# populationgenomics/cuKING

Hardware: AMD Instinct MI355X
Metric: sample-pairs/s (all-pairs KING) (higher is better)
Workload: dtype fp4 products, f32 accumulate (exact integers)

## Files before the change

### cuking_amd/csrc/king_common.h

```cpp
#ifndef CUKING_AMD_KING_COMMON_H_
#define CUKING_AMD_KING_COMMON_H_

#include <hip/hip_runtime.h>
#include <stdint.h>

#include "cuking_amd.h"
#include "king_submatrix.h"

namespace cuking {

constexpr uint32_t kLayoutWord = 0;
constexpr uint32_t kLayoutQuad = 1;
constexpr uint32_t kLayoutNibble = 2;
constexpr uint32_t kLayoutNibbleStats = 3;

struct PlaneGeometry {
  uint32_t num_rows, num_cols;
  uint32_t rows_padded, cols_padded;
  uint32_t col_base;
  uint32_t s_stride;
  uint32_t k_words;
  uint32_t diag;
};

// ... 65 lines not shown
  const uint32_t *tile_list_count;
  uint32_t tile_list_cap;
  const float2 *sample_stats;
  const uint4 *t2;
  uint32_t *filter_ctrl;
  unsigned long long *filter_totals;
  uint2 *cand_list;
  uint32_t cand_cap;
  uint32_t quadrant_cap;
  uint2 *dense_list;
  uint32_t dense_cap;
  uint32_t fsplit_parts, fsplit_first, fsplit_tile0;
  float4 *fsplit_slabs;
  uint32_t *fsplit_tickets;
  const uint32_t *check_steps;
  const float *prefix_u;
  const unsigned long long *cohort_sums;
  uint32_t check0, check1;
  uint32_t rotate, rotate_min_steps;
  uint32_t rotate_min_tiles;
  uint8_t *tile_done;
  const uint32_t *gate;
  uint32_t gate_count;
  const uint8_t *skip_tiles;
  uint64_t skip_base;
  const uint32_t *perm;
  uint32_t *codes_ready;
};

constexpr uint32_t kCheckEmitCap = 64;
constexpr uint32_t kNumCheckShares = 8;
constexpr uint32_t kCheckShares64[kNumCheckShares] = {8, 50, 53, 56, 58, 60, 61, 62};
constexpr uint32_t kNumPhases = 128;
constexpr uint32_t kPhasesPerShare = kNumPhases / 64;
constexpr uint32_t kNumCum = kNumPhases - 1;
__host__ __device__ inline uint32_t phase_step(uint32_t all_steps, uint32_t x) {
  return (uint32_t)((uint64_t)all_steps * x / kNumPhases);
}
__host__ __device__ inline uint32_t check_step_of(uint32_t all_steps, uint32_t k,
                                                  uint32_t min_steps = 64) {
  if (all_steps < min_steps) return 0;
  return phase_step(all_steps, kCheckShares64[k] * kPhasesPerShare);
}
constexpr uint32_t kFilterSplitSlabs = 256;
constexpr size_t kFilterSlabBytes = 256 * 256 * sizeof(float);
constexpr size_t kFilterTicketBytes = kFilterSplitSlabs * sizeof(uint32_t);
__host__ __device__ inline size_t plane_bytes(const PlaneGeometry &g,
                                              uint32_t layout) {
  const size_t base = (size_t)g.k_words * g.s_stride * (layout == kLayoutQuad ? 8 : 16);
  if (layout == kLayoutNibble) return base + base / 4;
  if (layout == kLayoutNibbleStats)
    return base + base / 4 + base / 2 + (size_t)g.s_stride * sizeof(float2) +
           (size_t)g.s_stride * kNumCum * sizeof(float) + 64 + 64 +
           64 + (size_t)g.s_stride * (4 + 8 + 4 * kNumCum + 16);
  return base;
}
__host__ __device__ inline const uint4 *plane_t2(const uint4 *planes, const PlaneGeometry &g) {
  return planes + (size_t)g.k_words * g.s_stride * 5 / 4;
}
__host__ __device__ inline const float2 *plane_stats(const uint4 *planes, const PlaneGeometry &g) {
  return reinterpret_cast<const float2 *>(planes + (size_t)g.k_words * g.s_stride * 7 / 4);
}
__host__ __device__ inline const float *plane_prefix_u(const uint4 *planes, const PlaneGeometry &g) {
  return reinterpret_cast<const float *>(plane_stats(planes, g) + g.s_stride);
}
__host__ __device__ inline const unsigned long long *plane_cohort_sums(const uint4 *planes,
                                                                       const PlaneGeometry &g) {
  return reinterpret_cast<const unsigned long long *>(plane_prefix_u(planes, g) +
                                                      (size_t)g.s_stride * kNumCum);
}

struct TiledVariant {
  const char *name;
  uint32_t tile;
  uint32_t k_chunk;
  uint32_t threads;
  uint32_t lds_bytes;
  uint32_t layout;
};

constexpr uint32_t kMfmaMaxSites = 1u << 24;

constexpr int kNumTiledVariants = 8;
constexpr int kMfmaVariant = 5;
constexpr int kMfmaN4Variant = 6;
constexpr uint32_t kMfmaN4MaxSites = 1u << 22;
constexpr int kMfmaN4Stages = 5;
constexpr uint32_t kMfmaN4LdsBytes = kMfmaN4Stages * 2 * 2 * 4 * 128 * 16;
static_assert(kMfmaN4LdsBytes <= 160 * 1024, "LDS of one CU");
constexpr int kMfmaFilterVariant = 7;
constexpr uint32_t kFilterTile = 256;
constexpr uint32_t kFilterLdsBytes = 5 * 2 * 2 * 2 * 256 * 16;
static_assert(kFilterLdsBytes <= 160 * 1024, "LDS of one CU");
constexpr uint32_t kFilterChunkTiles = 1u << 17;
constexpr uint32_t kFilterCandCap = 1u << 25;
constexpr uint32_t kFilterQuadrantCap = 384;
constexpr size_t kFilterCtrlBytes = 256;
constexpr uint32_t kCtrlCand = 0, kCtrlDense = 1, kCtrlDyn = 2, kCtrlFinished = 3,
                   kCtrlLeft = 4, kCtrlAllLeave = 5, kCtrlGate = 6;
constexpr uint32_t kCtrlStepTicks = 8, kCtrlPos = 16, kPosSlots = 16;
constexpr size_t kCtrlChunkBytes = (kCtrlPos + 8 * kPosSlots * 2) * 4;
constexpr uint32_t kTotalCand = 0, kTotalDense = 1, kTotalEarly = 2, kTotalRotated = 3;
constexpr uint32_t kNumTotals = 4;
__host__ __device__ inline const uint32_t *plane_check_steps(const uint4 *planes,
                                                             const PlaneGeometry &g) {
  return reinterpret_cast<const uint32_t *>(plane_cohort_sums(planes, g) + 8);
}
__host__ __device__ inline uint32_t *plane_flags(const uint4 *planes, const PlaneGeometry &g) {
  return const_cast<uint32_t *>(plane_check_steps(planes, g)) + 16;
}
__host__ __device__ inline uint32_t *plane_perm(const uint4 *planes, const PlaneGeometry &g) {
  return plane_flags(planes, g) + 16;
}
__host__ __device__ inline float2 *plane_tmp_stats(const uint4 *planes, const PlaneGeometry &g) {
  return reinterpret_cast<float2 *>(plane_perm(planes, g) + g.s_stride);
}
__host__ __device__ inline float *plane_tmp_prefix(const uint4 *planes, const PlaneGeometry &g) {
  return reinterpret_cast<float *>(plane_tmp_stats(planes, g) + g.s_stride);
}
__host__ __device__ inline uint32_t *plane_sort_words(const uint4 *planes, const PlaneGeometry &g) {
  return reinterpret_cast<uint32_t *>(plane_tmp_prefix(planes, g) +
                                      (size_t)g.s_stride * kNumCum);
}
constexpr uint32_t kNoSample = 0xFFFFFFFFu;

struct FilterScratchLayout {
  size_t tile_done, totals, tickets, cand, dense, slabs, bytes;
  uint32_t chunk_tiles, cand_entries;
};
inline FilterScratchLayout filter_scratch_layout(uint64_t tiles) {
  FilterScratchLayout l;
  l.chunk_tiles = (uint32_t)(tiles < kFilterChunkTiles ? (tiles ? tiles : 1) : kFilterChunkTiles);
  const uint64_t cand = (uint64_t)l.chunk_tiles * 4 * 64;
  l.cand_entries = (uint32_t)(cand < kFilterCandCap ? cand : kFilterCandCap);
  auto up = [](size_t x) { return (x + 255) / 256 * 256; };
  l.tile_done = kCtrlChunkBytes;
  l.totals = up(l.tile_done + l.chunk_tiles);
  l.tickets = l.totals + kFilterCtrlBytes;
  l.cand = l.tickets + kFilterTicketBytes;
  l.dense = l.cand + up((size_t)l.cand_entries * sizeof(uint2));
  l.slabs = l.dense + up((size_t)l.chunk_tiles * 4 * sizeof(uint2));
  l.bytes = l.slabs + kFilterSplitSlabs * kFilterSlabBytes;
  return l;
}
inline bool is_mfma_variant(int v) {
  return v == kMfmaVariant || v == kMfmaN4Variant || v == kMfmaFilterVariant;
}
constexpr int kMfmaStages = 6;
constexpr uint32_t kMfmaLdsBytes = kMfmaStages * 2 * 2 * 2 * 128 * 16;
constexpr uint32_t kMfmaParkBytes = 4 * 64 * 64 * 4;
static_assert(kMfmaLdsBytes + kMfmaParkBytes <= 160 * 1024, "LDS of one CU");
const TiledVariant &tiled_variant(int v);
hipError_t launch_tiled(int variant, bool full, const TiledArgs &args,
                        uint64_t num_tiles, hipStream_t stream);
hipError_t launch_mfma(bool full, bool nibble, const TiledArgs &args, uint64_t num_tiles,
                       uint32_t lds_bytes, hipStream_t stream);
hipError_t launch_mfma_list(const TiledArgs &args, uint32_t grid, hipStream_t stream);
hipError_t launch_mfma_gated(const TiledArgs &args, uint64_t num_units, uint32_t grid,
                             hipStream_t stream);
hipError_t launch_filter(const TiledArgs &args, uint64_t num_tiles, hipStream_t stream);
hipError_t launch_sample_stats(const uint64_t *d_bit_sets, uint32_t words_per_sample,
                               const PlaneGeometry &geo, uint4 *d_planes, uint32_t s_begin,
                               uint32_t s_end, hipStream_t stream);
void set_filter_check_min_steps(uint32_t steps);
uint32_t filter_check_min_steps();
size_t sort_temp_bytes_for(uint32_t n);
hipError_t launch_sample_order(const PlaneGeometry &geo, uint32_t words_per_sample,
                               uint4 *d_planes, uint32_t s_begin, uint32_t s_end, bool sort,
                               void *sort_temp, size_t sort_temp_bytes, hipStream_t stream);
hipError_t launch_prepare_nibbles(bool codes, bool t2, const uint64_t *d_bit_sets,
                                  uint32_t words_per_sample, const PlaneGeometry &geo,
                                  uint4 *d_planes, const uint32_t *perm, uint32_t s_tile_begin,
                                  uint32_t s_tile_end, const uint32_t *gate,
                                  const uint32_t *ready, hipStream_t stream);
hipError_t launch_mark_codes_ready(const uint32_t *gate, uint32_t *ready, hipStream_t stream);
// ... 45 lines not shown
```

### cuking_amd/csrc/king_filter.hip

```cpp
#include <hip/hip_runtime.h>
#include <stdio.h>

#include <atomic>
#include <stdlib.h>

#include "king_common.h"
#include "king_device.h"

#pragma clang diagnostic ignored "-Winline-asm"

namespace cuking {

namespace {

typedef int v8i __attribute__((ext_vector_type(8)));
typedef float v16f __attribute__((ext_vector_type(16)));

constexpr int kT = (int)kFilterTile;
constexpr int kUnits = 2;
constexpr int kStages = 5;
constexpr int kSliceU4 = kT;
constexpr int kStageU4 = 2 * 2 * kUnits * kSliceU4;
constexpr int kStageReqs = 4 * kUnits;
constexpr int kSyncVm = (kStages - 3) * kStageReqs + (kStageReqs - 2);
static_assert(kSyncVm < 64, "vmcnt is a 6-bit counter");
static_assert(kStages * kStageU4 * 16 == (int)kFilterLdsBytes, "LDS size");
constexpr int vmcnt_imm(int n) { return 0x0F70 | (n & 15) | ((n >> 4) << 14); }
constexpr uint32_t kNoPair = 0xFFFFFFFFu;

__device__ __forceinline__ uint32_t source_sample(const PlaneGeometry &geo, uint32_t ps) {
  if (geo.diag || ps < geo.rows_padded) return ps < geo.num_rows ? ps : kNoPair;
  const uint32_t c = ps - geo.col_base;
  return c < geo.num_cols ? geo.num_rows + c : kNoPair;
}

struct CheckWords {
  uint32_t w[kNumCheckShares];
};
constexpr uint32_t kStatsMaxSteps = kMfmaN4MaxSites / 256;
__global__ __launch_bounds__(256) void sample_stats_kernel(
    const uint64_t *__restrict__ bits, uint32_t words_per_sample, PlaneGeometry geo,
    float2 *__restrict__ stats, float *__restrict__ cum, unsigned long long *__restrict__ sums,
    uint32_t *__restrict__ steps_out, CheckWords cw, uint32_t s_begin, uint32_t s_end) {
  __shared__ uint8_t phase_of[kStatsMaxSteps];
  __shared__ int32_t phase_sum[4][kNumPhases];
  const uint32_t lane = threadIdx.x & 63, wave = threadIdx.x >> 6;
  if (blockIdx.x == 0 && threadIdx.x < kNumCheckShares) steps_out[threadIdx.x] = cw.w[threadIdx.x];
  const uint32_t all_steps = geo.k_words / 8;
  for (uint32_t st = threadIdx.x; st < all_steps; st += 256) {
    const uint32_t x = (kNumPhases * (st + 1) - 1) / all_steps;
    phase_of[st] = (uint8_t)(x < kNumPhases ? x : kNumPhases - 1);
  }
#pragma unroll
  for (uint32_t k = 0; k < kNumPhases / 64; ++k) phase_sum[wave][lane + 64 * k] = 0;
  __syncthreads();
  const uint32_t ps = s_begin + blockIdx.x * 4 + wave;
  if (ps >= s_end) return;
  const uint32_t src = source_sample(geo, ps);
  int32_t yc = 0, mc = 0, hc = 0;
  if (src != kNoPair) {
    const uint32_t n = words_per_sample / 2;
    const uint64_t *het = bits + (uint64_t)src * words_per_sample;
    const uint64_t *hom = het + n;
    constexpr uint32_t kAhead = 4;
    for (uint32_t w0 = 0; w0 < n; w0 += 64 * kAhead) {
      uint64_t h[kAhead], v[kAhead];
#pragma unroll
      for (uint32_t k = 0; k < kAhead; ++k) {
        const uint32_t w = w0 + 64 * k + lane;
        const bool in = w < n;
        h[k] = in ? het[w] : 0ull;
        v[k] = in ? hom[w] : 0ull;
      }
#pragma unroll
      for (uint32_t k = 0; k < kAhead; ++k) {
        const uint32_t w = w0 + 64 * k + lane;
        const bool in = w < n;
        const int32_t y = in ? __popcll(~h[k]) : 0;
        const int32_t m = __popcll(h[k] & v[k]);
        yc += y;
        mc += m;
        hc += __popcll(h[k] & ~v[k]);
        int32_t d = y - m;
        d += __shfl_xor(d, 1);
        d += __shfl_xor(d, 2);
        if ((lane & 3) == 0 && in) atomicAdd(&phase_sum[wave][phase_of[w >> 2]], d);
      }
    }
#pragma unroll
    for (int off = 32; off > 0; off >>= 1) {
      yc += __shfl_xor(yc, off);
      mc += __shfl_xor(mc, off);
      hc += __shfl_xor(hc, off);
    }
  }
  static_assert(kNumPhases == 128, "two phases per lane");
  const int32_t p0 = phase_sum[wave][2 * lane], p1 = phase_sum[wave][2 * lane + 1];
  int32_t run = p0 + p1;
#pragma unroll
  for (int off = 1; off < 64; off <<= 1) {
    const int32_t up = __shfl_up(run, off);
    if ((int)lane >= off) run += up;
  }
  cum[(size_t)(2 * lane) * geo.s_stride + ps] = (float)(run - p1);
  if (2 * lane + 1 < kNumCum) cum[(size_t)(2 * lane + 1) * geo.s_stride + ps] = (float)run;
  if (lane == 0) {
    stats[ps] = make_float2((float)(yc - mc), (float)hc);
    if (src != kNoPair && ((blockIdx.x & 15) == 0 || gridDim.x < 64)) {
      __hip_atomic_fetch_add(sums, 1ull, __ATOMIC_RELAXED, __HIP_MEMORY_SCOPE_AGENT);
      __hip_atomic_fetch_add(sums + 1, (unsigned long long)mc, __ATOMIC_RELAXED,
                             __HIP_MEMORY_SCOPE_AGENT);
      __hip_atomic_fetch_add(sums + 2, (unsigned long long)hc, __ATOMIC_RELAXED,
                             __HIP_MEMORY_SCOPE_AGENT);
    }
  }
}

__device__ __forceinline__ v16f mma(const v8i a, const v8i b, const v16f c) {
  return __builtin_amdgcn_mfma_scale_f32_32x32x64_f8f6f4(a, b, c, 4 , 4, 0, 0, 0, 0);
}

__device__ __forceinline__ v8i tfrag(const uint4 w, uint32_t mask) {
  v8i r = {0, 0, 0, 0, 0, 0, 0, 0};
  r[0] = (int)(w.x & mask);
  r[1] = (int)(w.y & mask);
  r[2] = (int)(w.z & mask);
  r[3] = (int)(w.w & mask);
  return r;
}

__device__ __forceinline__ uint4 shl2(const uint4 w) {
  return make_uint4(w.x << 2, w.y << 2, w.z << 2, w.w << 2);
}

#define F_ISSUE(SRC, DST, OFF)                                                 \
  asm volatile("s_mov_b32 m0, %0\n\t"                                          \
               "s_nop 0\n\t"                                                   \
               "global_load_lds_dwordx4 %1, %2 offset:" #OFF                   \
               :                                                               \
               : "s"(DST), "v"(lane16), "s"(SRC)                               \
               : "memory", "m0")

__device__ __forceinline__ int filter_tile(const TiledArgs &a, const uint32_t wg, uint4 *const lds) {
  uint32_t bid = wg;
  const bool split = a.fsplit_parts != 0 && wg >= a.fsplit_first;
  uint32_t part = 0, piece = 0;
  if (split) {
    piece = wg - a.fsplit_first;
    part = __builtin_amdgcn_readfirstlane(piece % a.fsplit_parts);
    bid = a.fsplit_tile0 + piece / a.fsplit_parts;
  } else
  if (a.dyn_tiles != 0 && wg >= a.launch_tiles) {
    uint32_t *slot = reinterpret_cast<uint32_t *>(lds);
    if (threadIdx.x == 0)
      *slot = __hip_atomic_fetch_add(a.filter_ctrl + kCtrlDyn, 1u, __ATOMIC_RELAXED,
                                     __HIP_MEMORY_SCOPE_AGENT);
    __syncthreads();
    const uint32_t t = __builtin_amdgcn_readfirstlane(*slot);
    __syncthreads();
    if (t >= a.dyn_tiles) return 1;
    bid = a.launch_tiles + t;
  } else if (a.xcd_chunk == 1) {
    const uint32_t x = bid & 7, j = bid >> 3;
    bid = (((j >> 5) * 8 + x) << 5) + (j & 31);
    if (bid >= a.launch_tiles) return 0;
  }
  bid = __builtin_amdgcn_readfirstlane(bid);
  uint32_t tr, tc;
  if (!decode_tile_space(a, a.tile_begin + bid, &tr, &tc)) return 0;
  tr = __builtin_amdgcn_readfirstlane(tr);
  tc = __builtin_amdgcn_readfirstlane(tc);

  const uint32_t lane = threadIdx.x & 63;
  const uint32_t wave = __builtin_amdgcn_readfirstlane(threadIdx.x >> 6);
  const uint32_t wy = wave >> 1, wx = wave & 1;
  uint32_t xcd_pos = 0;
  if (!split && a.tile_done != nullptr) {
    uint32_t *verdict = reinterpret_cast<uint32_t *>(lds);
    if (threadIdx.x == 0) {
      uint32_t leave = __hip_atomic_load(a.filter_ctrl + kCtrlAllLeave, __ATOMIC_RELAXED,
                                         __HIP_MEMORY_SCOPE_AGENT);
      if (leave == 0 && a.cohort_sums != nullptr && a.check_steps != nullptr) {
        const float ns = (float)a.cohort_sums[0], nm = (float)a.cohort_sums[1],
                    nh = (float)a.cohort_sums[2];
        if (ns > 0.f && nh > 0.f) {
// ... 16 lines not shown
        const uint32_t finished = __hip_atomic_load(a.filter_ctrl + kCtrlFinished, __ATOMIC_RELAXED,
                                                    __HIP_MEMORY_SCOPE_AGENT);
        if (finished >= 512 && 2 * dense_so_far > finished) {
          leave = 1;
          __hip_atomic_store(a.filter_ctrl + kCtrlAllLeave, 1u, __ATOMIC_RELAXED,
                             __HIP_MEMORY_SCOPE_AGENT);
          __hip_atomic_store(a.filter_ctrl + kCtrlGate, 1u, __ATOMIC_RELAXED,
                             __HIP_MEMORY_SCOPE_AGENT);
        }
      }
      verdict[0] = leave;
    }
    if (a.rotate == 1 && threadIdx.x < kPosSlots) {
      const uint32_t x = wg & 7;
      const unsigned long long said = __hip_atomic_load(
          reinterpret_cast<const unsigned long long *>(a.filter_ctrl + kCtrlPos) + x * kPosSlots +
              threadIdx.x,
          __ATOMIC_RELAXED, __HIP_MEMORY_SCOPE_AGENT);
      const uint32_t ticks16 = __hip_atomic_load(a.filter_ctrl + kCtrlStepTicks + x,
                                                 __ATOMIC_RELAXED, __HIP_MEMORY_SCOPE_AGENT);
      uint32_t pos = (uint32_t)(said >> 32);
      const uint32_t ago = (uint32_t)__builtin_amdgcn_s_memrealtime() - (uint32_t)said;
      if (said != 0 && ticks16 != 0 && ago < 16384u)
        pos += ago * 16u / ticks16;
      verdict[1 + threadIdx.x] = pos;
    }
    __syncthreads();
    const bool give_up = verdict[0] != 0;
    if (a.rotate == 1) {
#pragma unroll
      for (uint32_t k = 0; k < kPosSlots; ++k) xcd_pos = max(xcd_pos, verdict[1 + k]);
    }
    __syncthreads();
    if (give_up) {
      if (threadIdx.x == 0)
        __hip_atomic_fetch_add(a.filter_totals + kTotalDense, 4ull, __ATOMIC_RELAXED,
                               __HIP_MEMORY_SCOPE_AGENT);
      return 0;
    }
  }
  xcd_pos = __builtin_amdgcn_readfirstlane(xcd_pos);
  const uint32_t g = lane >> 5;
  const uint32_t lr = lane & 31;
  uint32_t lane16 = lane * 16;
  const uint32_t s_stride = a.geo.s_stride;
  const uint32_t all_steps = a.geo.k_words / (4 * kUnits);
  const uint32_t k_first = __builtin_amdgcn_readfirstlane(
      split ? part * all_steps / a.fsplit_parts : 0u);
  const uint32_t num_steps = __builtin_amdgcn_readfirstlane(
      split ? (part + 1) * all_steps / a.fsplit_parts - k_first : all_steps);
  const uint4 *g_rows = a.t2 + (uint64_t)tr * kT;
  const uint4 *g_cols = a.t2 + a.geo.col_base + (uint64_t)tc * kT;

  uint32_t mT;
  asm volatile("s_mov_b32 %0, 0xcccccccc" : "=s"(mT));

  const uint32_t dma_side = wave >> 1, dma_h = wave & 1;
  const uint32_t row_bytes = s_stride * 16;
  const char *const g_wave = reinterpret_cast<const char *>(
      (dma_side ? g_cols : g_rows) + ((uint64_t)2 * kUnits * k_first + kUnits * dma_h) * s_stride);
  const uint32_t l_wave = (uint32_t)(uintptr_t)(lds_void_ptr)(
      lds + ((dma_side * 2 + dma_h) * kUnits) * kSliceU4);
  struct Addr { const char *src; uint32_t dst; };
  const uint32_t kstep_bytes = 2 * kUnits * row_bytes;
  const char *seg_src = g_wave;
  uint32_t seg_steps = num_steps;
  uint32_t seg_wrap = 0xFFFFFFFFu;
  auto addr_of = [&](uint32_t step, uint32_t buf) {
    Addr pa;
    if (step >= seg_steps) step = seg_steps - 1;
    const int32_t rel = (int32_t)step - (int32_t)(step >= seg_wrap ? all_steps : 0u);
    pa.src = seg_src + (int64_t)rel * (int64_t)kstep_bytes;
    pa.dst = l_wave + buf * (kStageU4 * 16);
    asm volatile("" : "+s"(pa.src), "+s"(pa.dst));
    return pa;
  };
  auto addr_next = [&](const Addr &cur, uint32_t step, uint32_t buf) {
    Addr pa;
    const int32_t adv = (int32_t)(step < seg_steps ? 1u : 0u) -
                        (int32_t)(step == seg_wrap ? all_steps : 0u);
    pa.src = cur.src + (int64_t)adv * (int64_t)kstep_bytes;
    pa.dst = l_wave + buf * (kStageU4 * 16);
    asm volatile("" : "+s"(pa.src), "+s"(pa.dst));
    return pa;
  };
#define F_ISSUE4(PA, C)                                                        \
  {                                                                            \
    const char *src_ = (PA).src + (C) * row_bytes;                             \
    const uint32_t dst_ = (PA).dst + (C) * (kSliceU4 * 16);                    \
    F_ISSUE(src_, dst_, 0);                                                    \
    F_ISSUE(src_, dst_, 1024);                                                 \
    F_ISSUE(src_, dst_, 2048);                                                 \
    F_ISSUE(src_, dst_, 3072);                                                 \
  }

  v16f acc[4][4];
#pragma unroll
  for (int bi = 0; bi < 4; ++bi)
#pragma unroll
    for (int bj = 0; bj < 4; ++bj)
#pragma unroll
      for (int r = 0; r < 16; ++r) acc[bi][bj][r] = 0.f;

  uint32_t row_off = ((0 * 2 + g) * kUnits) * kSliceU4 + wy * 128 + lr;
  uint32_t col_off = ((1 * 2 + g) * kUnits) * kSliceU4 + wx * 128 + lr;
  asm volatile("" : "+v"(row_off), "+v"(col_off), "+v"(lane16));
  v8i FA[2][4], FB[2][4];
  uint4 RAW[8];
#define F_READ(K, BUF, C)                                                      \
  RAW[K] = lds[(BUF) * kStageU4 + ((K) < 4 ? row_off : col_off) + (C) * kSliceU4 + ((K) & 3) * 32];
#define F_PIN4(W) asm volatile("" : "+v"((W).x), "+v"((W).y), "+v"((W).z), "+v"((W).w));
#define F_PINF(F) asm volatile("" : "+v"((F)[0]), "+v"((F)[1]), "+v"((F)[2]), "+v"((F)[3]));
#define F_BUILD_B(NXT, K)                                                      \
  F_PIN4(RAW[K])                                                               \
  if ((K) < 4) {                                                               \
    FA[NXT][(K) & 3] = tfrag(RAW[K], mT);                                      \
    F_PINF(FA[NXT][(K) & 3])                                                   \
  } else {                                                                     \
    FB[NXT][(K) & 3] = tfrag(RAW[K], mT);                                      \
    F_PINF(FB[NXT][(K) & 3])                                                   \
  }
#define F_BUILD_A(NXT, K)                                                      \
  F_PIN4(RAW[K])                                                               \
  if ((K) < 4) {                                                               \
    FA[NXT][(K) & 3] = tfrag(shl2(RAW[K]), mT);                                \
    F_PINF(FA[NXT][(K) & 3])                                                   \
  } else {                                                                     \
    FB[NXT][(K) & 3] = tfrag(shl2(RAW[K]), mT);                                \
    F_PINF(FB[NXT][(K) & 3])                                                   \
  }
#define F_MMA(CUR, BI, BJ) acc[BI][BJ] = mma(FA[CUR][BI], FB[CUR][BJ], acc[BI][BJ]);
#define F_BAR __builtin_amdgcn_sched_barrier(0);
#define F_SLICE_B(CUR, NXT, PA, DC, OFF0, OFF1)                                \
  {                                                                            \
    const char *src_ = (PA).src + (DC) * row_bytes;                            \
    const uint32_t dst_ = (PA).dst + (DC) * (kSliceU4 * 16);                   \
    F_ISSUE(src_, dst_, OFF0);                                                 \
    F_MMA(CUR, 0, 0) F_BAR                                                     \
    F_BUILD_A(NXT, 0) F_MMA(CUR, 0, 1) F_BAR                                   \
    F_MMA(CUR, 0, 2) F_BAR                                                     \
    F_BUILD_A(NXT, 1) F_MMA(CUR, 0, 3) F_BAR                                   \
    F_MMA(CUR, 1, 0) F_BAR                                                     \
    F_BUILD_A(NXT, 2) F_MMA(CUR, 1, 1) F_BAR                                   \
    F_MMA(CUR, 1, 2) F_BAR                                                     \
    F_BUILD_A(NXT, 3) F_MMA(CUR, 1, 3) F_BAR                                   \
    F_ISSUE(src_, dst_, OFF1);                                                 \
    F_MMA(CUR, 2, 0) F_BAR                                                     \
    F_BUILD_A(NXT, 4) F_MMA(CUR, 2, 1) F_BAR                                   \
    F_MMA(CUR, 2, 2) F_BAR                                                     \
    F_BUILD_A(NXT, 5) F_MMA(CUR, 2, 3) F_BAR                                   \
    F_MMA(CUR, 3, 0) F_BAR                                                     \
    F_BUILD_A(NXT, 6) F_MMA(CUR, 3, 1) F_BAR                                   \
    F_MMA(CUR, 3, 2) F_BAR                                                     \
    F_BUILD_A(NXT, 7) F_MMA(CUR, 3, 3) F_BAR                                   \
  }
#define F_SLICE_A(CUR, NXT, RBUF, RC, SYNC, PA, DC, OFF0, OFF1)                \
  {                                                                            \
    if (SYNC) {                                                                \
      __builtin_amdgcn_s_waitcnt(vmcnt_imm(kSyncVm));                          \
      __syncthreads();                                                         \
    }                                                                          \
    const char *src_ = (PA).src + (DC) * row_bytes;                            \
    const uint32_t dst_ = (PA).dst + (DC) * (kSliceU4 * 16);                   \
    F_READ(0, RBUF, RC) F_READ(1, RBUF, RC)                                    \
    F_ISSUE(src_, dst_, OFF0);                                                 \
    F_MMA(CUR, 0, 0) F_MMA(CUR, 0, 1) F_BAR                                    \
    F_READ(2, RBUF, RC) F_READ(3, RBUF, RC)                                    \
    F_MMA(CUR, 0, 2) F_MMA(CUR, 0, 3) F_BAR                                    \
    F_READ(4, RBUF, RC) F_READ(5, RBUF, RC)                                    \
    F_ISSUE(src_, dst_, OFF1);                                                 \
    F_MMA(CUR, 1, 0) F_MMA(CUR, 1, 1) F_BAR                                    \
    F_READ(6, RBUF, RC) F_READ(7, RBUF, RC)                                    \
    F_MMA(CUR, 1, 2) F_MMA(CUR, 1, 3) F_BAR                                    \
    F_BUILD_B(NXT, 0) F_MMA(CUR, 2, 0) F_BAR                                   \
    F_BUILD_B(NXT, 1) F_MMA(CUR, 2, 1) F_BAR                                   \
    F_BUILD_B(NXT, 2) F_MMA(CUR, 2, 2) F_BAR                                   \
    F_BUILD_B(NXT, 3) F_MMA(CUR, 2, 3) F_BAR                                   \
    F_BUILD_B(NXT, 4) F_MMA(CUR, 3, 0) F_BAR                                   \
    F_BUILD_B(NXT, 5) F_MMA(CUR, 3, 1) F_BAR                                   \
    F_BUILD_B(NXT, 6) F_MMA(CUR, 3, 2) F_BAR                                   \
    F_BUILD_B(NXT, 7) F_MMA(CUR, 3, 3) F_BAR                                   \
  }
#define F_KSTEP                                                                \
  {                                                                            \
// ... 24 lines not shown
        phase = (bid * 37u + 11u) & (kNumPhases - 1);
      } else {
        phase = (a.rotate - 3u) & (kNumPhases - 1);
      }
      k0 = phase_step(all_steps, phase);
      start_abs = base + k0;
      wrap = k0 != 0 ? all_steps - k0 : 0u;
    }
    float kappa = -1.f;
    {
      const float ns = (float)a.cohort_sums[0], nm = (float)a.cohort_sums[1],
                  nh = (float)a.cohort_sums[2];
      if (ns > 0.f && nh > 0.f) {
        const float sites = 256.f * (float)all_steps;
        const float m = nm / (ns * sites), h = nh / (ns * sites);
        kappa = m * (1.f + m / (2.f * h * (1.f - m))) + 4.6f * rsqrtf(sites) + 0.003f;
      }
    }
    auto steps_of = [&](uint32_t share) {
      const uint32_t hi = phase + share * kPhasesPerShare;
      return hi <= kNumPhases ? phase_step(all_steps, hi) - k0
                              : (all_steps - k0) + phase_step(all_steps, hi - kNumPhases);
    };
    if ((a.check0 == 2 || (a.check0 == 1 && kappa > 0.7f * a.kin_threshold)) &&
        a.check_steps[0] != 0)
      chk0 = steps_of(kCheckShares64[0]);
    const uint32_t sw1 = a.check1 & 0xFFu;
    if (sw1 >= 2) {
      entry1 = sw1 - 2;
    } else if (sw1 == 1 && kappa >= 0.f) {
      const float f64 = 64.f * (1.f - 2.f * a.kin_threshold) / (1.f - 2.f * kappa);
      if (f64 <= 62.f) {
        share1 = (uint32_t)ceilf(f64);
        if (share1 < 32) share1 = 32;
        entry1 = 1;
      }
    }
#pragma unroll
    for (uint32_t k = 1; k < kNumCheckShares; ++k)
      if (sw1 >= 2 && k == entry1) share1 = kCheckShares64[k];
    if (share1 != 0 && a.check_steps[entry1] != 0) chk1 = steps_of(share1);
    if (chk0 >= num_steps) chk0 = 0;
    if (chk1 >= num_steps || chk1 <= chk0) chk1 = 0;
  }
  chk0 = __builtin_amdgcn_readfirstlane(chk0);
  chk1 = __builtin_amdgcn_readfirstlane(chk1);
  share1 = __builtin_amdgcn_readfirstlane(share1);
  phase = __builtin_amdgcn_readfirstlane(phase);
  k0 = __builtin_amdgcn_readfirstlane(k0);
  wrap = __builtin_amdgcn_readfirstlane(wrap);
  start_abs = __builtin_amdgcn_readfirstlane(start_abs);
  auto prefix_u_of = [&](uint32_t share, size_t idx, float total) {
    const uint32_t hi = phase + share * kPhasesPerShare;
    const uint32_t xb = hi > kNumPhases ? hi - kNumPhases : hi;
    float u = hi > kNumPhases ? total : 0.f;
    if (xb == kNumPhases)
      u += total;
    else if (xb != 0)
      u += a.prefix_u[(size_t)(xb - 1) * s_stride + idx];
    if (phase != 0) u -= a.prefix_u[(size_t)(phase - 1) * s_stride + idx];
    return u;
  };
  unsigned long long *const pos_word =
      reinterpret_cast<unsigned long long *>(a.filter_ctrl + kCtrlPos) +
      (wg & 7) * kPosSlots + ((wg >> 3) & (kPosSlots - 1));
  uint32_t *const ticks_word = a.filter_ctrl + kCtrlStepTicks + (wg & 7);
  const uint32_t t_start = a.rotate == 1 ? (uint32_t)__builtin_amdgcn_s_memrealtime() : 0u;
#define F_PUBLISH(STEPS)                                                       \
  if (a.rotate == 1 && wave == 0) {                                            \
    const uint32_t now_ = (uint32_t)__builtin_amdgcn_s_memrealtime();          \
    const unsigned long long val_ =                                            \
        ((unsigned long long)(start_abs + (STEPS)) << 32) | now_;              \
     \
    const uint32_t t16_ = (STEPS) >= 32 ? (now_ - t_start) * 16u / (STEPS) : 0u; \
    const uint32_t zero_ = 0;                                                  \
    unsigned long long save_;                                                  \
    asm volatile("s_mov_b64 %0, exec\n\t"                                      \
                 "s_mov_b64 exec, 1\n\t"                                       \
                 "global_store_dwordx2 %1, %2, %3\n\t"                         \
                 "s_mov_b64 exec, %0"                                          \
                 : "=&s"(save_)                                                \
                 : "v"(zero_), "v"(val_), "s"(pos_word)                        \
                 : "memory");                                                  \
    if (t16_ != 0)                                                             \
      asm volatile("s_mov_b64 %0, exec\n\t"                                    \
                   "s_mov_b64 exec, 1\n\t"                                     \
                   "global_store_dword %1, %2, %3\n\t"                         \
                   "s_mov_b64 exec, %0"                                        \
                   : "=&s"(save_)                                              \
                   : "v"(zero_), "v"(t16_), "s"(ticks_word)                    \
                   : "memory");                                                \
  }

  uint32_t seg_first = 0;
  bool left = false, left_forecast = false, left_emit = false;
#pragma nounroll
  while (true) {
    uint32_t seg_end = num_steps;
    if (chk1 > seg_first) seg_end = chk1;
    if (chk0 > seg_first) seg_end = chk0;
    seg_end = __builtin_amdgcn_readfirstlane(seg_end);
    seg_steps = seg_end - seg_first;
    const uint32_t seg_k = seg_first >= wrap && wrap != 0 ? seg_first - wrap : k0 + seg_first;
    seg_src = g_wave + (uint64_t)seg_k * kstep_bytes;
    seg_wrap = __builtin_amdgcn_readfirstlane(
        wrap > seg_first && wrap < seg_end ? wrap - seg_first : 0xFFFFFFFFu);
    asm volatile("" : "+s"(seg_src), "+s"(seg_steps), "+s"(seg_wrap));

#pragma unroll
    for (int st = 0; st < kStages - 1; ++st) {
      const Addr p0 = addr_of(st, st);
      F_ISSUE4(p0, 0)
      F_ISSUE4(p0, 1)
// ... 1 lines not shown
    __builtin_amdgcn_s_waitcnt(vmcnt_imm((kStages - 2) * kStageReqs));
    __syncthreads();
#pragma unroll
    for (int k = 0; k < 8; ++k) {
      F_READ(k, 0, 0)
    }
#pragma unroll
    for (int k = 0; k < 8; ++k) {
      F_BUILD_B(0, k)
    }
    uint32_t buf = 0;
    Addr pa = addr_of(kStages - 1, kStages - 1);
    uint32_t step = 0;
    while (step + 1 < seg_steps) {
      F_KSTEP
      F_KSTEP
    }
    if (step < seg_steps) F_KSTEP
    __builtin_amdgcn_s_waitcnt(0x0F70);
    __syncthreads();
    F_PUBLISH(seg_end)
    if (seg_end == num_steps) break;

    const bool forecast = seg_end == chk0;
    const float scale = forecast ? (float)kCheckShares64[0] * (1.f / 64.f) : 1.f;
    float2 *const ck_rows = reinterpret_cast<float2 *>(lds);
    float2 *const ck_cols = ck_rows + kT;
    uint32_t *const ck_words = reinterpret_cast<uint32_t *>(ck_cols + kT);
    {
      const uint32_t share = forecast ? kCheckShares64[0] : share1;
      const float thr_f = forecast ? a.kin_threshold + 3.66f * rsqrtf(256.f * (float)all_steps)
                                   : a.kin_threshold;
      const float t = 2.f - 4.f * thr_f;
      const size_t ir = (size_t)tr * kT + threadIdx.x;
      const size_t ic = (size_t)a.geo.col_base + (size_t)tc * kT + threadIdx.x;
      const float2 sr = a.sample_stats[ir], sc = a.sample_stats[ic];
      ck_rows[threadIdx.x] = make_float2(prefix_u_of(share, ir, sr.x), scale * fmaf(t, sr.y, 8.f));
      ck_cols[threadIdx.x] = make_float2(prefix_u_of(share, ic, sc.x), scale * fmaf(t, sc.y, 8.f));
    }
    __syncthreads();
    const uint32_t emit_cap = (a.check1 >> 8) & 0xFFu;
    uint32_t cnt = 0;
    {
      float2 cc[4];
#pragma unroll
      for (int bj = 0; bj < 4; ++bj) cc[bj] = ck_cols[wx * 128 + bj * 32 + lr];
#pragma unroll
      for (int bi = 0; bi < 4; ++bi)
#pragma unroll
        for (int r = 0; r < 16; ++r) {
          const float2 cr = ck_rows[wy * 128 + bi * 32 + (r & 3) + 8 * (r >> 2) + 4 * g];
#pragma unroll
          for (int bj = 0; bj < 4; ++bj)
            cnt += fmaf(-0.5f, acc[bi][bj][r], cr.x + cc[bj].x) < fminf(cr.y, cc[bj].y) ? 1u : 0u;
        }
    }
#pragma unroll
    for (int off = 32; off > 0; off >>= 1) cnt += __shfl_xor(cnt, off);
    if (lane == 0)
      ck_words[wave] = forecast ? (cnt > 2 * a.quadrant_cap ? 1u : 0u)
                                : (cnt > emit_cap ? emit_cap + 1 : cnt);
    __syncthreads();
    uint32_t found = forecast ? ck_words[0] + ck_words[1] + ck_words[2] + ck_words[3]
                              : max(max(ck_words[0], ck_words[1]), max(ck_words[2], ck_words[3]));
    found = __builtin_amdgcn_readfirstlane(found);
    __syncthreads();
    if (forecast ? found >= 3 : found <= emit_cap) {
      left = true;
      left_forecast = forecast;
      left_emit = !forecast && found != 0;
      break;
    }
    seg_first = seg_end;
  }
#undef F_KSTEP
#undef F_SLICE_A
#undef F_SLICE_B
#undef F_BAR
#undef F_MMA
#undef F_BUILD_A
#undef F_BUILD_B
#undef F_PIN4
#undef F_PINF
#undef F_READ
#undef F_ISSUE4
#undef F_PUBLISH
  if (left && left_emit && threadIdx.x == 0)
    __hip_atomic_fetch_add(a.filter_totals + kTotalEarly, 1ull, __ATOMIC_RELAXED,
                           __HIP_MEMORY_SCOPE_AGENT);
  if (phase != 0 && threadIdx.x == 0)
    __hip_atomic_fetch_add(a.filter_totals + kTotalRotated, 1ull, __ATOMIC_RELAXED,
                           __HIP_MEMORY_SCOPE_AGENT);
  if (left && !left_emit) {
    if (threadIdx.x == 0) {
      __hip_atomic_fetch_add(a.filter_ctrl + kCtrlFinished, 4u, __ATOMIC_RELAXED,
                             __HIP_MEMORY_SCOPE_AGENT);
      if (left_forecast) {
        __hip_atomic_fetch_add(a.filter_ctrl + kCtrlLeft, 4u, __ATOMIC_RELAXED,
                               __HIP_MEMORY_SCOPE_AGENT);
        __hip_atomic_store(a.filter_ctrl + kCtrlGate, 1u, __ATOMIC_RELAXED,
                           __HIP_MEMORY_SCOPE_AGENT);
        __hip_atomic_fetch_add(
            a.filter_totals + kTotalDense, 4ull,
            __ATOMIC_RELAXED, __HIP_MEMORY_SCOPE_AGENT);
      } else {
        a.tile_done[bid] = 1;
        __hip_atomic_fetch_add(
// ... 48 lines not shown
    __syncthreads();
    if (!last) return 0;
    const uint32_t first_piece = piece - part;
    for (uint32_t p = 0; p < a.fsplit_parts; ++p) {
      if (p == part) continue;
      const float4 *src = a.fsplit_slabs + (size_t)(first_piece + p) * kSlabU4 + threadIdx.x;
#pragma unroll
      for (int bi = 0; bi < 4; ++bi)
#pragma unroll
        for (int bj = 0; bj < 4; ++bj)
#pragma unroll
          for (int r4 = 0; r4 < 4; ++r4) {
            const float4 v = src[((bi * 4 + bj) * 4 + r4) * 256];
            acc[bi][bj][4 * r4] += v.x;
            acc[bi][bj][4 * r4 + 1] += v.y;
            acc[bi][bj][4 * r4 + 2] += v.z;
            acc[bi][bj][4 * r4 + 3] += v.w;
          }
    }
  }

  float2 *const st_rows = reinterpret_cast<float2 *>(lds);
  float2 *const st_cols = st_rows + kT;
  {
    const float t = 2.f - 4.f * a.kin_threshold;
    const size_t ir = (size_t)tr * kT + threadIdx.x;
    const size_t ic = (size_t)a.geo.col_base + (size_t)tc * kT + threadIdx.x;
    float2 r = a.sample_stats[ir];
    float2 c = a.sample_stats[ic];
    if (left_emit) {
      r.x = prefix_u_of(share1, ir, r.x);
      c.x = prefix_u_of(share1, ic, c.x);
    }
    r.y = fmaf(t, r.y, 8.f);
    c.y = fmaf(t, c.y, 8.f);
    st_rows[threadIdx.x] = r;
    st_cols[threadIdx.x] = c;
  }
  __syncthreads();
  float2 sc[4];
#pragma unroll
  for (int bj = 0; bj < 4; ++bj) sc[bj] = st_cols[wx * 128 + bj * 32 + lr];

  {
    float best = -1.f;
#pragma unroll
    for (int bi = 0; bi < 4; ++bi)
#pragma unroll
      for (int r = 0; r < 16; ++r) {
        const float2 sr = st_rows[wy * 128 + bi * 32 + (r & 3) + 8 * (r >> 2) + 4 * g];
#pragma unroll
        for (int bj = 0; bj < 4; ++bj)
          best = fmaxf(best, fminf(sr.y, sc[bj].y) -
                                 fmaf(-0.5f, acc[bi][bj][r], sr.x + sc[bj].x));
      }
    if (__ballot(best > 0.f) == 0) {
      if (lane == 0)
        __hip_atomic_fetch_add(a.filter_ctrl + kCtrlFinished, 1u, __ATOMIC_RELAXED, __HIP_MEMORY_SCOPE_AGENT);
      return 0;
    }
  }
  if (lane == 0)
    __hip_atomic_fetch_add(a.filter_ctrl + kCtrlFinished, 1u, __ATOMIC_RELAXED, __HIP_MEMORY_SCOPE_AGENT);

  uint32_t total = 0, base = 0, run = 0;
#pragma nounroll
  for (int pass = 0; pass < 2; ++pass) {
    uint32_t tr_p = tr, tc_p = tc;
    asm volatile("" : "+s"(tr_p), "+s"(tc_p));
#pragma unroll
    for (int bi = 0; bi < 4; ++bi) {
#pragma unroll
      for (int r = 0; r < 16; ++r) {
        const uint32_t row = wy * 128 + bi * 32 + (r & 3) + 8 * (r >> 2) + 4 * g;
        const float2 sr = st_rows[row];
        const uint32_t li = tr_p * kT + row;
#pragma unroll
        for (int bj = 0; bj < 4; ++bj) {
          const uint32_t lj = tc_p * kT + wx * 128 + bj * 32 + lr;
          const bool valid = li < a.geo.num_rows && lj < a.geo.num_cols &&
                             a.i_begin + li < a.j_begin + lj;
          const float x_lb = fmaf(-0.5f, acc[bi][bj][r], sr.x + sc[bj].x);
          const bool cand = valid && x_lb < fminf(sr.y, sc[bj].y);
          const unsigned long long b = __ballot(cand);
          if (b != 0) {
            if (pass == 0) {
              total += (uint32_t)__popcll(b);
            } else {
              const uint32_t before = __builtin_amdgcn_mbcnt_hi(
                  (uint32_t)(b >> 32), __builtin_amdgcn_mbcnt_lo((uint32_t)b, 0u));
              if (cand) a.cand_list[base + run + before] = make_uint2(li, lj);
              run += (uint32_t)__popcll(b);
            }
          }
        }
      }
    }
    if (pass == 0) {
      if (total == 0) break;
      bool dense = total > a.quadrant_cap;
      if (!dense) {
        uint32_t got = 0;
        if (lane == 0) {
          got = __hip_atomic_fetch_add(a.filter_ctrl, total, __ATOMIC_RELAXED,
                                       __HIP_MEMORY_SCOPE_AGENT);
          __hip_atomic_fetch_add(a.filter_totals + kTotalCand,
                                 (unsigned long long)total, __ATOMIC_RELAXED,
                                 __HIP_MEMORY_SCOPE_AGENT);
        }
        base = (uint32_t)__builtin_amdgcn_readfirstlane(got);
        if (base >= a.cand_cap || total > a.cand_cap - base) {
          for (uint32_t k = base + lane; k < a.cand_cap; k += 64)
            a.cand_list[k] = make_uint2(kNoPair, kNoPair);
          dense = true;
        }
      }
      if (dense) {
        if (lane == 0) {
          const uint32_t slot = __hip_atomic_fetch_add(a.filter_ctrl + kCtrlDense, 1u, __ATOMIC_RELAXED,
                                                       __HIP_MEMORY_SCOPE_AGENT);
          if (slot < a.dense_cap) a.dense_list[slot] = make_uint2(2 * tr + wy, 2 * tc + wx);
          __hip_atomic_fetch_add(a.filter_totals + kTotalDense, 1ull,
                                 __ATOMIC_RELAXED, __HIP_MEMORY_SCOPE_AGENT);
        }
        break;
      }
    }
  }
  return 0;
}

__global__ __launch_bounds__(256, 1) void king_filter_kernel(const TiledArgs a) {
  extern __shared__ uint4 lds[];
  (void)filter_tile(a, blockIdx.x, lds);
}
// ... 197 lines not shown
```

### cuking_amd/csrc/king_kernels.hip

```cpp
#include <hip/hip_runtime.h>

#include "king_common.h"
#include "king_device.h"

#pragma clang diagnostic ignored "-Winline-asm"

namespace cuking {

namespace {

constexpr int kPrepSamples = 64;
constexpr int kPrepWords = 16;

__global__ __launch_bounds__(256) void prepare_planes_kernel(
    const uint64_t *__restrict__ bits, uint32_t words_per_sample,
    PlaneGeometry geo, uint4 *__restrict__ planes, uint32_t s_tile_begin) {
  __shared__ uint64_t het_lds[kPrepSamples][kPrepWords + 1];
  __shared__ uint64_t hom_lds[kPrepSamples][kPrepWords + 1];

  const uint32_t plane_words = words_per_sample / 2;
  const uint32_t s0 = (s_tile_begin + blockIdx.x) * kPrepSamples;
  const uint32_t w0 = blockIdx.y * kPrepWords;

#pragma unroll
// ... 154 lines not shown
  }
  __syncthreads();

  if constexpr (CODES) {
#pragma unroll
  for (int it = 0; it < kPrepSamples * kNibWords * 2 / 256; ++it) {
    const uint32_t idx = it * 256 + threadIdx.x;
    const uint32_t krow = idx / kPrepSamples, s = idx % kPrepSamples;
    const uint32_t k = w0 * 2 + krow;
    if (k >= geo.k_words || s0 + s >= geo.s_stride) continue;
    const uint32_t shift = (krow & 1) * 32;
    const uint32_t het = (uint32_t)(het_lds[s][krow >> 1] >> shift);
    const uint32_t hom = (uint32_t)(hom_lds[s][krow >> 1] >> shift);
    uint32_t out[4];
#pragma unroll
    for (int d = 0; d < 4; ++d) {
      const uint32_t hs = spread8(het >> (8 * d)), ms = spread8(hom >> (8 * d));
      const uint32_t H = hs & ~ms;
      const uint32_t D = 0x11111111u ^ (hs & ms);
      const uint32_t Y = 0x11111111u ^ hs;
      const uint32_t A = ms & ~hs;
      out[d] = H | (D << 1) | (Y << 2) | (A << 3);
    }
    planes[(uint64_t)k * geo.s_stride + s0 + s] = make_uint4(out[0], out[1], out[2], out[3]);
  }
  uint4 *hetq = planes + (uint64_t)geo.k_words * geo.s_stride;
  constexpr int kQuads = kNibWords / 2;
#pragma unroll
  for (int it = 0; it < kQuads * kPrepSamples / 256; ++it) {
    const uint32_t idx = it * 256 + threadIdx.x;
    const uint32_t s = idx % kPrepSamples, ql = idx / kPrepSamples;
    const uint32_t q = w0 / 2 + ql;
    if (q * 4 >= geo.k_words || s0 + s >= geo.s_stride) continue;
    const uint64_t lo = het_lds[s][2 * ql], hi = het_lds[s][2 * ql + 1];
    hetq[(uint64_t)q * geo.s_stride + s0 + s] =
        make_uint4((uint32_t)lo, (uint32_t)(lo >> 32), (uint32_t)hi, (uint32_t)(hi >> 32));
  }
  }
  if constexpr (T2) {
    uint4 *t2 = const_cast<uint4 *>(plane_t2(planes, geo));
#pragma unroll
    for (int it = 0; it < kNibWords * kPrepSamples / 256; ++it) {
      const uint32_t idx = it * 256 + threadIdx.x;
      const uint32_t s = idx % kPrepSamples, ul = idx / kPrepSamples;
      const uint32_t u = w0 + ul;
      if (u * 2 >= geo.k_words || s0 + s >= geo.s_stride) continue;
      const uint64_t het = het_lds[s][ul], hom = hom_lds[s][ul];
      uint32_t out[4];
#pragma unroll
      for (int d = 0; d < 4; ++d) {
        const uint32_t h_lo = (uint32_t)(het >> (8 * d)), m_lo = (uint32_t)(hom >> (8 * d));
        const uint32_t h_hi = (uint32_t)(het >> (32 + 8 * d)), m_hi = (uint32_t)(hom >> (32 + 8 * d));
        const uint32_t y_lo = spread8(~h_lo), a_lo = spread8(m_lo & ~h_lo);
        const uint32_t y_hi = spread8(~h_hi), a_hi = spread8(m_hi & ~h_hi);
        out[d] = (a_lo << 3) | (y_lo << 2) | (a_hi << 1) | y_hi;
      }
      t2[(uint64_t)u * geo.s_stride + s0 + s] = make_uint4(out[0], out[1], out[2], out[3]);
    }
  }
}

template <int TIT, int TJT, int RI, int RJ, int KC, int KU, int MINW, bool FULL,
          bool PHASED = false>
__global__ __launch_bounds__(TIT *TJT, MINW) void king_tiled_kernel(
    const TiledArgs a) {
  constexpr int TILE = TIT * RI;
  static_assert(TILE == TJT * RJ, "square tiles only");
  constexpr int NT = TIT * TJT;
  constexpr int NW = NT / 64;
  constexpr int SEG = TILE / 64;
  constexpr int WAVE_ROWS = 2 * KC * SEG;
  static_assert(WAVE_ROWS % NW == 0, "rows must split evenly over waves");
  constexpr int PER_WAVE = WAVE_ROWS / NW;

  extern __shared__ uint4 lds[];

  const uint64_t t = a.tile_begin + blockIdx.x;
  uint32_t tr, tc;
  if (!decode_tile(a, t, &tr, &tc)) return;

  const uint32_t lane = threadIdx.x & 63;
  const uint32_t wave = __builtin_amdgcn_readfirstlane(threadIdx.x >> 6);
  const uint32_t ti = threadIdx.x % TIT;
  const uint32_t tj = threadIdx.x / TIT;

  const uint4 *g_rows = a.planes + (uint64_t)tr * TILE;
  const uint4 *g_cols = a.planes + a.geo.col_base + (uint64_t)tc * TILE;
  const uint32_t s_stride = a.geo.s_stride;
  const uint32_t num_chunks = a.geo.k_words / KC;

  auto issue_chunk = [&](uint32_t chunk, uint32_t buf) {
#pragma unroll
    for (int r = 0; r < PER_WAVE; ++r) {
      const uint32_t wr = wave * PER_WAVE + r;
      const uint32_t side = wr / (KC * SEG);
      const uint32_t rem = wr % (KC * SEG);
      const uint32_t kc = rem / SEG, seg = rem % SEG;
      const uint4 *src = (side ? g_cols : g_rows) +
                         (uint64_t)(chunk * KC + kc) * s_stride + seg * 64 +
                         lane;
      uint4 *dst = lds + ((buf * 2 + side) * KC + kc) * TILE + seg * 64;
      if (PHASED) {
        const uint32_t lds_addr = (uint32_t)(uintptr_t)(lds_void_ptr)dst;
        asm volatile(
            "s_mov_b32 m0, %0\n\t"
            "s_nop 0\n\t"
            "global_load_lds_dwordx4 %1, off"
            :
// ... 453 lines not shown
```

### cuking_amd/csrc/king_sort.hip

```cpp
#include <hip/hip_runtime.h>

#include <hipcub/hipcub.hpp>

#include "king_common.h"

namespace cuking {

namespace {

__global__ void sort_keys_kernel(const float2 *__restrict__ tmp_stats, uint32_t begin, uint32_t n,
                                 float stored_sites, uint32_t *__restrict__ keys,
                                 uint32_t *__restrict__ vals) {
  const uint32_t p = blockIdx.x * blockDim.x + threadIdx.x;
  if (p >= n) return;
  const float2 st = tmp_stats[begin + p];
  const float missing = 0.5f * (stored_sites - st.y - st.x);
  uint32_t key = (uint32_t)(missing * 64.f / stored_sites);
  keys[p] = key > 255u ? 255u : key;
  vals[p] = begin + p;
}

__global__ void identity_order_kernel(uint32_t begin, uint32_t n, uint32_t *__restrict__ vals) {
  const uint32_t p = blockIdx.x * blockDim.x + threadIdx.x;
  if (p < n) vals[p] = begin + p;
}

__global__ void apply_order_kernel(PlaneGeometry geo, uint32_t begin, uint32_t end, uint32_t n,
                                   const uint32_t *__restrict__ order,
                                   const float2 *__restrict__ tmp_stats,
                                   const float *__restrict__ tmp_prefix,
                                   uint32_t *__restrict__ perm, float2 *__restrict__ stats,
                                   float *__restrict__ prefix) {
  const uint32_t p = begin + blockIdx.x * blockDim.x + threadIdx.x;
  if (p >= end) return;
  if (p - begin >= n) {
    perm[p] = kNoSample;
    stats[p] = make_float2(0.f, 0.f);
#pragma unroll
    for (uint32_t c = 0; c < kNumCum; ++c) prefix[(size_t)c * geo.s_stride + p] = 0.f;
    return;
  }
  const uint32_t src = order[p - begin];
  perm[p] = (geo.diag || src < geo.rows_padded) ? src : geo.num_rows + (src - geo.col_base);
  stats[p] = tmp_stats[src];
#pragma unroll 7
  for (uint32_t c = 0; c < kNumCum; ++c)
    prefix[(size_t)c * geo.s_stride + p] = tmp_prefix[(size_t)c * geo.s_stride + src];
}

}

size_t sort_temp_bytes_for(uint32_t n) {
  size_t bytes = 0;
  uint32_t *nil = nullptr;
  if (n == 0) return 0;
  (void)hipcub::DeviceRadixSort::SortPairs(nullptr, bytes, nil, nil, nil, nil, (int)n, 0, 8);
  return (bytes + 255) / 256 * 256;
}

hipError_t launch_sample_order(const PlaneGeometry &geo, uint32_t words_per_sample,
                               uint4 *d_planes, uint32_t s_begin, uint32_t s_end, bool sort,
                               void *sort_temp, size_t sort_temp_bytes, hipStream_t stream) {
  if (s_end > geo.s_stride) s_end = geo.s_stride;
  if (s_begin >= s_end) return hipSuccess;
  const float2 *tmp_stats = plane_tmp_stats(d_planes, geo);
  const float *tmp_prefix = plane_tmp_prefix(d_planes, geo);
  uint32_t *perm = plane_perm(d_planes, geo);
  float2 *stats = const_cast<float2 *>(plane_stats(d_planes, geo));
  float *prefix = const_cast<float *>(plane_prefix_u(d_planes, geo));
  uint32_t *words = plane_sort_words(d_planes, geo);
  const float stored_sites = 32.f * (float)words_per_sample;
  struct Side { uint32_t begin, end, real_end; };
  Side sides[2];
  int num_sides = 0;
  if (geo.diag) {
    sides[num_sides++] = {0, geo.rows_padded, geo.num_rows};
  } else {
    sides[num_sides++] = {0, geo.rows_padded, geo.num_rows};
    sides[num_sides++] = {geo.col_base, geo.col_base + geo.cols_padded, geo.col_base + geo.num_cols};
  }
  for (int k = 0; k < num_sides; ++k) {
    const uint32_t b = s_begin > sides[k].begin ? s_begin : sides[k].begin;
    const uint32_t e = s_end < sides[k].end ? s_end : sides[k].end;
    if (b >= e) continue;
    const uint32_t real_e = e < sides[k].real_end ? e : sides[k].real_end;
    const uint32_t n = real_e > b ? real_e - b : 0;
    uint32_t *keys_in = words + b, *keys_out = words + geo.s_stride + b;
    uint32_t *vals_in = words + 2 * (size_t)geo.s_stride + b;
    uint32_t *vals_out = words + 3 * (size_t)geo.s_stride + b;
    const uint32_t *order = vals_in;
    if (n != 0) {
      if (sort) {
        sort_keys_kernel<<<dim3((n + 255) / 256), dim3(256), 0, stream>>>(
            tmp_stats, b, n, stored_sites, keys_in, vals_in);
        hipError_t e0 = hipGetLastError();
        if (e0 != hipSuccess) return e0;
        size_t bytes = sort_temp_bytes;
// ... 20 lines not shown
```

Before: 37.52 billion.

## Re-encode filter fp4 operands to drop per-fragment shift and fold bias into stats

Changes the second-plane nibble encoding so the filter MFMA A/B fragments can be built with a plain mask instead of a shift-then-mask. It uses MFMA block scaling on one half of the K slice. The lower-bound algebra is rewritten with a -8x coefficient, and per-sample stats and prefix sums absorb a constant bias term computed in the stats kernel. An extra cumulative row is stored for this. This aims to remove the per-fragment shift ALU work in the hot loop. In exchange it adds more stats work, a wider scratch layout and subtler exactness requirements on float sums.

After: 39.05 billion, median of 6. 1.04x the previous value.

```diff
diff --git a/cuking_amd/csrc/king_common.h b/cuking_amd/csrc/king_common.h
--- a/cuking_amd/csrc/king_common.h
+++ b/cuking_amd/csrc/king_common.h
@@ -141,7 +141,7 @@
   if (layout == kLayoutNibbleStats)
     return base + base / 4 + base / 2 + (size_t)g.s_stride * sizeof(float2) +
            (size_t)g.s_stride * kNumCum * sizeof(float) + 64 + 64 +
-           64 + (size_t)g.s_stride * (4 + 8 + 4 * kNumCum + 16);
+           64 + (size_t)g.s_stride * (4 + 8 + 4 * (kNumCum + 1) + 16);
   return base;
 }
 __host__ __device__ inline const uint4 *plane_t2(const uint4 *planes, const PlaneGeometry &g) {
@@ -174,6 +174,7 @@
 constexpr int kMfmaVariant = 5;
 constexpr int kMfmaN4Variant = 6;
 constexpr uint32_t kMfmaN4MaxSites = 1u << 22;
+static_assert(4ull * kMfmaN4MaxSites <= (1ull << 24), "filter kernel: exact float sums");
 constexpr int kMfmaN4Stages = 5;
 constexpr uint32_t kMfmaN4LdsBytes = kMfmaN4Stages * 2 * 2 * 4 * 128 * 16;
 static_assert(kMfmaN4LdsBytes <= 160 * 1024, "LDS of one CU");
@@ -209,7 +210,7 @@
 }
 __host__ __device__ inline uint32_t *plane_sort_words(const uint4 *planes, const PlaneGeometry &g) {
   return reinterpret_cast<uint32_t *>(plane_tmp_prefix(planes, g) +
-                                      (size_t)g.s_stride * kNumCum);
+                                      (size_t)g.s_stride * (kNumCum + 1));
 }
 constexpr uint32_t kNoSample = 0xFFFFFFFFu;
 
diff --git a/cuking_amd/csrc/king_filter.hip b/cuking_amd/csrc/king_filter.hip
--- a/cuking_amd/csrc/king_filter.hip
+++ b/cuking_amd/csrc/king_filter.hip
@@ -57,7 +57,7 @@
   const uint32_t ps = s_begin + blockIdx.x * 4 + wave;
   if (ps >= s_end) return;
   const uint32_t src = source_sample(geo, ps);
-  int32_t yc = 0, mc = 0, hc = 0;
+  int32_t yc = 0, mc = 0, hc = 0, sa = 0;
   if (src != kNoPair) {
     const uint32_t n = words_per_sample / 2;
     const uint64_t *het = bits + (uint64_t)src * words_per_sample;
@@ -81,7 +81,10 @@
         yc += y;
         mc += m;
         hc += __popcll(h[k] & ~v[k]);
-        int32_t d = y - m;
+        const uint64_t hom_a = in ? ~h[k] & 0xFFFFFFFF00000000ull : 0ull;
+        const int32_t t_a = __popcll(hom_a & ~v[k]) - __popcll(hom_a & v[k]);
+        sa += t_a;
+        int32_t d = y - m + 2 * t_a;
         d += __shfl_xor(d, 1);
         d += __shfl_xor(d, 2);
         if ((lane & 3) == 0 && in) atomicAdd(&phase_sum[wave][phase_of[w >> 2]], d);
@@ -92,6 +95,7 @@
       yc += __shfl_xor(yc, off);
       mc += __shfl_xor(mc, off);
       hc += __shfl_xor(hc, off);
+      sa += __shfl_xor(sa, off);
     }
   }
   static_assert(kNumPhases == 128, "two phases per lane");
@@ -102,10 +106,14 @@
     const int32_t up = __shfl_up(run, off);
     if ((int)lane >= off) run += up;
   }
-  cum[(size_t)(2 * lane) * geo.s_stride + ps] = (float)(run - p1);
-  if (2 * lane + 1 < kNumCum) cum[(size_t)(2 * lane + 1) * geo.s_stride + ps] = (float)run;
+  cum[(size_t)(2 * lane) * geo.s_stride + ps] =
+      (float)(run - p1 + (int32_t)(128u * phase_step(all_steps, 2 * lane + 1)));
+  if (2 * lane + 1 < kNumCum)
+    cum[(size_t)(2 * lane + 1) * geo.s_stride + ps] =
+        (float)(run + (int32_t)(128u * phase_step(all_steps, 2 * lane + 2)));
   if (lane == 0) {
     stats[ps] = make_float2((float)(yc - mc), (float)hc);
+    cum[(size_t)kNumCum * geo.s_stride + ps] = (float)(yc - mc + 2 * sa + (int32_t)(128u * all_steps));
     if (src != kNoPair && ((blockIdx.x & 15) == 0 || gridDim.x < 64)) {
       __hip_atomic_fetch_add(sums, 1ull, __ATOMIC_RELAXED, __HIP_MEMORY_SCOPE_AGENT);
       __hip_atomic_fetch_add(sums + 1, (unsigned long long)mc, __ATOMIC_RELAXED,
@@ -118,6 +126,10 @@
 
 __device__ __forceinline__ v16f mma(const v8i a, const v8i b, const v16f c) {
   return __builtin_amdgcn_mfma_scale_f32_32x32x64_f8f6f4(a, b, c, 4 , 4, 0, 0, 0, 0);
+}
+
+__device__ __forceinline__ v16f mma_scaled(const v8i a, const v8i b, const v16f c, const int scale) {
+  return __builtin_amdgcn_mfma_scale_f32_32x32x64_f8f6f4(a, b, c, 4 , 4, 0, scale, 0, scale);
 }
 
 __device__ __forceinline__ v8i tfrag(const uint4 w, uint32_t mask) {
@@ -127,10 +139,6 @@
   r[2] = (int)(w.z & mask);
   r[3] = (int)(w.w & mask);
   return r;
-}
-
-__device__ __forceinline__ uint4 shl2(const uint4 w) {
-  return make_uint4(w.x << 2, w.y << 2, w.z << 2, w.w << 2);
 }
 
 #define F_ISSUE(SRC, DST, OFF)                                                 \
@@ -253,8 +261,11 @@
   const uint4 *g_rows = a.t2 + (uint64_t)tr * kT;
   const uint4 *g_cols = a.t2 + a.geo.col_base + (uint64_t)tc * kT;
 
-  uint32_t mT;
+  uint32_t mT, mA;
   asm volatile("s_mov_b32 %0, 0xcccccccc" : "=s"(mT));
+  asm volatile("s_mov_b32 %0, 0x33333333" : "=s"(mA));
+  int scaleB;
+  asm volatile("v_mov_b32 %0, 0x7d7d7d7d" : "=v"(scaleB));
 
   const uint32_t dma_side = wave >> 1, dma_h = wave & 1;
   const uint32_t row_bytes = s_stride * 16;
@@ -324,13 +335,15 @@
 #define F_BUILD_A(NXT, K)                                                      \
   F_PIN4(RAW[K])                                                               \
   if ((K) < 4) {                                                               \
-    FA[NXT][(K) & 3] = tfrag(shl2(RAW[K]), mT);                                \
+    FA[NXT][(K) & 3] = tfrag(RAW[K], mA);                                      \
     F_PINF(FA[NXT][(K) & 3])                                                   \
   } else {                                                                     \
-    FB[NXT][(K) & 3] = tfrag(shl2(RAW[K]), mT);                                \
+    FB[NXT][(K) & 3] = tfrag(RAW[K], mA);                                      \
     F_PINF(FB[NXT][(K) & 3])                                                   \
   }
-#define F_MMA(CUR, BI, BJ) acc[BI][BJ] = mma(FA[CUR][BI], FB[CUR][BJ], acc[BI][BJ]);
+#define F_MMA(CUR, BI, BJ)                                                     \
+  acc[BI][BJ] = (CUR) == 0 ? mma_scaled(FA[CUR][BI], FB[CUR][BJ], acc[BI][BJ], scaleB) \
+                           : mma(FA[CUR][BI], FB[CUR][BJ], acc[BI][BJ]);
 #define F_BAR __builtin_amdgcn_sched_barrier(0);
 #define F_SLICE_B(CUR, NXT, PA, DC, OFF0, OFF1)                                \
   {                                                                            \
@@ -461,13 +474,11 @@
   start_abs = __builtin_amdgcn_readfirstlane(start_abs);
   auto prefix_u_of = [&](uint32_t share, size_t idx, float total) {
     const uint32_t hi = phase + share * kPhasesPerShare;
-    const uint32_t xb = hi > kNumPhases ? hi - kNumPhases : hi;
-    float u = hi > kNumPhases ? total : 0.f;
-    if (xb == kNumPhases)
-      u += total;
-    else if (xb != 0)
-      u += a.prefix_u[(size_t)(xb - 1) * s_stride + idx];
+    float u = hi >= kNumPhases ? total
+              : hi != 0        ? a.prefix_u[(size_t)(hi - 1) * s_stride + idx]
+                               : 0.f;
     if (phase != 0) u -= a.prefix_u[(size_t)(phase - 1) * s_stride + idx];
+    if (hi > kNumPhases) u += a.prefix_u[(size_t)(hi - kNumPhases - 1) * s_stride + idx];
     return u;
   };
   unsigned long long *const pos_word =
@@ -575,7 +586,7 @@
           const float2 cr = ck_rows[wy * 128 + bi * 32 + (r & 3) + 8 * (r >> 2) + 4 * g];
 #pragma unroll
           for (int bj = 0; bj < 4; ++bj)
-            cnt += fmaf(-0.5f, acc[bi][bj][r], cr.x + cc[bj].x) < fminf(cr.y, cc[bj].y) ? 1u : 0u;
+            cnt += fmaf(-8.f, acc[bi][bj][r], cr.x) + cc[bj].x < fminf(cr.y, cc[bj].y) ? 1u : 0u;
         }
     }
 #pragma unroll
@@ -730,7 +741,7 @@
 #pragma unroll
         for (int bj = 0; bj < 4; ++bj)
           best = fmaxf(best, fminf(sr.y, sc[bj].y) -
-                                 fmaf(-0.5f, acc[bi][bj][r], sr.x + sc[bj].x));
+                                 (fmaf(-8.f, acc[bi][bj][r], sr.x) + sc[bj].x));
       }
     if (__ballot(best > 0.f) == 0) {
       if (lane == 0)
@@ -758,7 +769,7 @@
           const uint32_t lj = tc_p * kT + wx * 128 + bj * 32 + lr;
           const bool valid = li < a.geo.num_rows && lj < a.geo.num_cols &&
                              a.i_begin + li < a.j_begin + lj;
-          const float x_lb = fmaf(-0.5f, acc[bi][bj][r], sr.x + sc[bj].x);
+          const float x_lb = fmaf(-8.f, acc[bi][bj][r], sr.x) + sc[bj].x;
           const bool cand = valid && x_lb < fminf(sr.y, sc[bj].y);
           const unsigned long long b = __ballot(cand);
           if (b != 0) {
diff --git a/cuking_amd/csrc/king_kernels.hip b/cuking_amd/csrc/king_kernels.hip
--- a/cuking_amd/csrc/king_kernels.hip
+++ b/cuking_amd/csrc/king_kernels.hip
@@ -230,8 +230,8 @@
         const uint32_t h_lo = (uint32_t)(het >> (8 * d)), m_lo = (uint32_t)(hom >> (8 * d));
         const uint32_t h_hi = (uint32_t)(het >> (32 + 8 * d)), m_hi = (uint32_t)(hom >> (32 + 8 * d));
         const uint32_t y_lo = spread8(~h_lo), a_lo = spread8(m_lo & ~h_lo);
-        const uint32_t y_hi = spread8(~h_hi), a_hi = spread8(m_hi & ~h_hi);
-        out[d] = (a_lo << 3) | (y_lo << 2) | (a_hi << 1) | y_hi;
+        const uint32_t r_hi = spread8(~h_hi & ~m_hi), n_hi = spread8(h_hi);
+        out[d] = (a_lo << 3) | (y_lo << 2) | (r_hi << 1) | n_hi;
       }
       t2[(uint64_t)u * geo.s_stride + s0 + s] = make_uint4(out[0], out[1], out[2], out[3]);
     }
diff --git a/cuking_amd/csrc/king_sort.hip b/cuking_amd/csrc/king_sort.hip
--- a/cuking_amd/csrc/king_sort.hip
+++ b/cuking_amd/csrc/king_sort.hip
@@ -34,15 +34,17 @@
   const uint32_t p = begin + blockIdx.x * blockDim.x + threadIdx.x;
   if (p >= end) return;
   if (p - begin >= n) {
+    const uint32_t all_steps = geo.k_words / 8;
     perm[p] = kNoSample;
-    stats[p] = make_float2(0.f, 0.f);
+    stats[p] = make_float2((float)(128u * all_steps), 0.f);
 #pragma unroll
-    for (uint32_t c = 0; c < kNumCum; ++c) prefix[(size_t)c * geo.s_stride + p] = 0.f;
+    for (uint32_t c = 0; c < kNumCum; ++c)
+      prefix[(size_t)c * geo.s_stride + p] = (float)(128u * phase_step(all_steps, c + 1));
     return;
   }
   const uint32_t src = order[p - begin];
   perm[p] = (geo.diag || src < geo.rows_padded) ? src : geo.num_rows + (src - geo.col_base);
-  stats[p] = tmp_stats[src];
+  stats[p] = make_float2(tmp_prefix[(size_t)kNumCum * geo.s_stride + src], tmp_stats[src].y);
 #pragma unroll 7
   for (uint32_t c = 0; c < kNumCum; ++c)
     prefix[(size_t)c * geo.s_stride + p] = tmp_prefix[(size_t)c * geo.s_stride + src];
```
